# mathematiguy/pypardis

Measured on AMD Instinct MI355X. Metric: points clustered/sec (whole node), 100M 3-D pts, 1/2/4/8 GPUs; % HBM roofline, higher is better.
Workload: dtype f32 coords, f64 predicate

## Files before the change

### pypardis_amd/csrc/engine.hip

```cpp
#include <cstring>
#include <rocprim/rocprim.hpp>
#ifndef PD_SORT_ROCPRIM
#define PD_SORT_ROCPRIM 0
#endif

#include <algorithm>
#include <type_traits>
#include <cmath>
#include <cstring>
#include <vector>

#include "compact.hpp"
#include "internal.hpp"
#include "pred.hpp"
#include "rsort.hpp"
#include "scan.hpp"
#include "stream.hpp"
#include "uf.hpp"

namespace pd {
namespace {

#ifndef PD_CHECK_BOUNDS
#define PD_CHECK_BOUNDS 0
// ... 526 lines not shown
__global__ __launch_bounds__(kBlock) void cell_tile_kernel(const K* __restrict__ keys, uint64_t R,
                                                           uint32_t* __restrict__ tile_cnt) {
    uint32_t st[4];
    uint64_t kv[4];
    const uint64_t r0 = ((uint64_t)blockIdx.x * kBlock + threadIdx.x) * 4;
    const uint32_t t = block_sum_u32(cell_starts4<K>(keys, R, r0, st, kv));
    if (threadIdx.x == 0) tile_count_out(tile_cnt, t);
}

template <typename K>
__global__ __launch_bounds__(kBlock) void cell_write_kernel(const K* __restrict__ keys, uint64_t R,
                                                            const uint64_t* __restrict__ tile_off,
                                                            uint32_t* __restrict__ cstart,
                                                            K* __restrict__ ckeys,
                                                            uint32_t* __restrict__ ncells) {
    uint32_t st[4];
    uint64_t kv[4];
    const uint64_t r0 = ((uint64_t)blockIdx.x * kBlock + threadIdx.x) * 4;
    uint32_t btot;
    const uint32_t c = cell_starts4<K>(keys, R, r0, st, kv);
    uint32_t cid = (uint32_t)tile_off[blockIdx.x] + block_excl_scan(c, btot);
#pragma unroll
    for (int q = 0; q < 4; ++q) {
        if (st[q]) {
            cstart[cid] = (uint32_t)(r0 + q);
            ckeys[cid] = (K)kv[q];
        }
        cid += st[q];
        if (r0 + q == R - 1) {
            cstart[cid] = (uint32_t)R;
            *ncells = cid;
        }
    }
}

template <typename WT>
__device__ __forceinline__ WT shfl_up_w(WT x, int o) {
    if constexpr (sizeof(WT) == 4) return (WT)__shfl_up((int)x, o, 64);
    else return (WT)__shfl_up((long long)x, o, 64);
}
template <typename WT>
__device__ __forceinline__ WT shfl_down_w(WT x, int o) {
    if constexpr (sizeof(WT) == 4) return (WT)__shfl_down((int)x, o, 64);
    else return (WT)__shfl_down((long long)x, o, 64);
}
template <typename WT>
__device__ __forceinline__ WT shfl_w(WT x, int l) {
    if constexpr (sizeof(WT) == 4) return (WT)__shfl((int)x, l, 64);
    else return (WT)__shfl((long long)x, l, 64);
}

template <typename K, int SH, bool W32>
__global__ __launch_bounds__(kBlock) void dir_bits_kernel(const K* __restrict__ ckeys,
                                                          const uint32_t* __restrict__ ncells,
                                                          uint4* __restrict__ dir) {
    const uint32_t c = blockIdx.x * kBlock + threadIdx.x;
    const uint32_t nc = *ncells;
    if (c - (uint32_t)(threadIdx.x & 63) >= nc) return;
    const bool in = c < nc;
    using WT = std::conditional_t<W32, uint32_t, uint64_t>;
    const uint64_t k = in ? ((uint64_t)ckeys[c] >> SH) : ~0ull;
    const WT word = (WT)(k >> 6);
    unsigned long long v = in ? (1ull << (k & 63)) : 0ull;
    const int lane = threadIdx.x & 63;
#pragma unroll
    for (int o = 1; o < 64; o <<= 1) {
        const WT wo = shfl_up_w(word, o);
        const unsigned long long vo = (unsigned long long)__shfl_up((long long)v, o, 64);
        if (lane >= o && wo == word) v |= vo;
    }
    const WT wn = shfl_down_w(word, 1);
    const bool last = lane == 63 || wn != word;
    if (in && last) atomicOr(reinterpret_cast<unsigned long long*>(dir + (uint64_t)word), v);
}

template <typename K, bool W32>
__global__ __launch_bounds__(kBlock) void word_write_kernel(const K* __restrict__ ckeys,
                                                            const uint32_t* __restrict__ ncells,
                                                            const uint4* __restrict__ pages,
                                                            uint4* __restrict__ words) {
    const uint32_t c = blockIdx.x * kBlock + threadIdx.x;
    const uint32_t nc = *ncells;
    if (c - (uint32_t)(threadIdx.x & 63) >= nc) return;
    const bool in = c < nc;
    using WT = std::conditional_t<W32, uint32_t, uint64_t>;
    const uint64_t k = in ? (uint64_t)ckeys[c] : ~0ull;
    const WT word = (WT)(k >> 6);
    unsigned long long v = in ? (1ull << (k & 63)) : 0ull;
    const int lane = threadIdx.x & 63;
#pragma unroll
    for (int o = 1; o < 64; o <<= 1) {
        const WT wo = shfl_down_w(word, o);
        const unsigned long long vo = (unsigned long long)__shfl_down((long long)v, o, 64);
        if (lane + o < 64 && wo == word) v |= vo;
    }
    const WT wp = shfl_up_w(word, 1);
    const WT w63 = shfl_w(word, 63);
    const uint32_t cb = c - (uint32_t)lane;
    unsigned long long vx = 0;
    if (cb + 64 < nc && (WT)((uint64_t)ckeys[cb + 64] >> 6) == w63) {
        const uint32_t c2 = cb + 64 + (uint32_t)lane;
        const uint64_t k2 = c2 < nc ? (uint64_t)ckeys[c2] : ~0ull;
        vx = c2 < nc && (WT)(k2 >> 6) == w63 ? 1ull << (k2 & 63) : 0ull;
#pragma unroll
        for (int o = 32; o > 0; o >>= 1) vx |= (unsigned long long)__shfl_xor((long long)vx, o, 64);
    }
    if (!in) return;
    bool first = c == 0;
    if (!first) first = lane ? wp != word : (WT)((uint64_t)ckeys[c - 1] >> 6) != word;
    bool occ;
    const uint64_t slot = page_slot(pages[(uint64_t)word >> 6], (uint64_t)word, occ);
    if (first) {
        if (w63 == word) v |= vx;
        words[slot] = make_uint4((uint32_t)v, (uint32_t)(v >> 32), c, 0u);
    }
    if (c == nc - 1) words[slot + 1] = make_uint4(0u, 0u, nc, 0u);
}

__device__ __forceinline__ uint32_t dir_popc4(const uint4* __restrict__ dir, uint64_t W,
                                              uint64_t w0, uint32_t (&pc)[4]) {
    uint32_t t = 0;
#pragma unroll
    for (int q = 0; q < 4; ++q) {
        pc[q] = 0;
        if (w0 + q < W) {
            const uint4 d = dir[w0 + q];
            pc[q] = (uint32_t)__popc(d.x) + (uint32_t)__popc(d.y);
        }
        t += pc[q];
    }
    return t;
}

__global__ __launch_bounds__(kBlock) void dir_tile_kernel(const uint4* __restrict__ dir, uint64_t W,
                                                          uint32_t* __restrict__ tile_cnt) {
    uint32_t pc[4];
    const uint32_t t =
        block_sum_u32(dir_popc4(dir, W, ((uint64_t)blockIdx.x * kBlock + threadIdx.x) * 4, pc));
    if (threadIdx.x == 0) tile_count_out(tile_cnt, t);
}

__global__ __launch_bounds__(kBlock) void dir_write_kernel(uint4* __restrict__ dir, uint64_t W,
                                                           const uint64_t* __restrict__ tile_off) {
    uint32_t pc[4], btot;
    const uint64_t w0 = ((uint64_t)blockIdx.x * kBlock + threadIdx.x) * 4;
    uint32_t z = (uint32_t)tile_off[blockIdx.x] + block_excl_scan(dir_popc4(dir, W, w0, pc), btot);
#pragma unroll
    for (int q = 0; q < 4; ++q) {
        if (w0 + q < W) dir[w0 + q].z = z;
        z += pc[q];
    }
}

constexpr int kSubTiles = 4;
#ifndef PD_ROOTS_SUB
#define PD_ROOTS_SUB 4
#endif
constexpr int kRootSub = PD_ROOTS_SUB;
constexpr int kRootLists = 64, kRootCntStride = 32;
__global__ __launch_bounds__(kBlock) void init_kernel(uint32_t R, const uint8_t* __restrict__ core,
                                                      const uint32_t* __restrict__ mn,
                                                      int use_mn, uint32_t* __restrict__ par,
                                                      uint32_t* __restrict__ gmin,
                                                      uint32_t* __restrict__ wroot, uint64_t W,
                                                      uint32_t* __restrict__ kbits, uint64_t NW) {
#pragma unroll
    for (int q = 0; q < kSubTiles; ++q) {
        const uint64_t r64 = ((uint64_t)blockIdx.x * kSubTiles + q) * kBlock + threadIdx.x;
        if (r64 < W) wroot[r64] = kNone;
        if (r64 < NW) kbits[r64] = 0u;
        if (r64 >= R) continue;
        const uint32_t r = (uint32_t)r64;
        gmin[r] = kNone;
        uint32_t p = kNone;
        if (core[r] & 1) {
            p = r;
            if (use_mn) {
                const uint2 m = reinterpret_cast<const uint2*>(mn)[r];
                if (m.x < r && (core[m.x] & 1))
                    p = m.x;
                else if (m.y < r && (core[m.y] & 1))
                    p = m.y;
            }
        }
        par[r] = p;
    }
}

struct LinkStats {
    uint32_t cand = 0, hit = 0, core = 0, same = 0, find_same = 0, unions = 0;
};

__global__ __launch_bounds__(kBlock) void rep_kernel(const uint32_t* __restrict__ list,
                                                     const uint32_t* __restrict__ count,
                                                     const uint32_t* __restrict__ vals,
                                                     const uint32_t* __restrict__ par,
                                                     uint32_t* __restrict__ rep) {
    const uint32_t nl = *count;
    for (uint32_t i = blockIdx.x * kBlock + threadIdx.x; i < nl; i += gridDim.x * kBlock) {
        const uint32_t r = list[i];
        if (par[r] != kNone) atomicMin(rep + (vals[r] & kIdMask), r);
    }
}

__global__ __launch_bounds__(kBlock) void merge_kernel(const uint32_t* __restrict__ list,
                                                       const uint32_t* __restrict__ count,
                                                       const uint32_t* __restrict__ vals,
                                                       const uint32_t* __restrict__ rep,
                                                       uint32_t* __restrict__ par) {
    const uint32_t nl = *count;
    const int lane = threadIdx.x & 63;
    for (uint32_t b0 = blockIdx.x * kBlock; b0 < nl; b0 += gridDim.x * kBlock) {
        const uint32_t i = b0 + threadIdx.x;
        uint32_t ra = kNone, rb = kNone;
        if (i < nl) {
            const uint32_t r = list[i];
            if (ld_rlx(par + r) != kNone) {
                const uint32_t q = rep[vals[r] & kIdMask];
                if (q != r) {
                    ra = uf_find(par, r);
                    rb = uf_find(par, q);
                    if (ra > rb) {
                        const uint32_t t = ra;
                        ra = rb;
                        rb = t;
                    }
                    if (ra == rb) ra = rb = kNone;
                }
            }
        }
        const uint32_t pa = (uint32_t)__shfl_up((int)ra, 1, 64);
        const uint32_t pb = (uint32_t)__shfl_up((int)rb, 1, 64);
        const bool same = lane > 0 && pa == ra && pb == rb;
        if (ra != kNone && !same) uf_unite(par, ra, rb);
    }
}

__global__ __launch_bounds__(kBlock) void roots_kernel(uint32_t R, const uint32_t* __restrict__ vals,
                                                       const uint32_t* __restrict__ gid,
                                                       uint32_t* __restrict__ par,
                                                       uint32_t* __restrict__ gmin,
                                                       uint32_t* __restrict__ rlist,
                                                       uint32_t* __restrict__ rcnt, uint32_t seg,
                                                       uint32_t* __restrict__ counts, int stats) {
    uint32_t ncore = 0;
    uint32_t rr[kRootSub], x0[kRootSub], root[kRootSub], pt[kRootSub];
    bool core[kRootSub];
#pragma unroll
    for (int q = 0; q < kRootSub; ++q) {
        rr[q] = (blockIdx.x * kRootSub + q) * kBlock + threadIdx.x;
        x0[q] = rr[q] < R ? par[rr[q]] : kNone;
        core[q] = x0[q] != kNone;
    }
#pragma unroll
    for (int q = 0; q < kRootSub; ++q) {
        root[q] = core[q] ? par[x0[q]] : 0u;
        pt[q] = core[q] ? (vals[rr[q]] & kIdMask) : kNone;
    }
    bool more[kRootSub];
#pragma unroll
    for (int q = 0; q < kRootSub; ++q) more[q] = core[q] && root[q] != x0[q];
    while (true) {
        bool any = false;
#pragma unroll
        for (int q = 0; q < kRootSub; ++q) any |= more[q];
        if (!__any(any)) break;
        uint32_t p[kRootSub];
#pragma unroll
        for (int q = 0; q < kRootSub; ++q) p[q] = more[q] ? par[root[q]] : root[q];
#pragma unroll
        for (int q = 0; q < kRootSub; ++q) {
            if (p[q] == root[q]) more[q] = false;
            root[q] = p[q];
        }
    }
#pragma unroll
    for (int q = 0; q < kRootSub; ++q) {
        if (!core[q]) continue;
        if (root[q] != x0[q]) par[rr[q]] = root[q];
        if (gid) pt[q] = gid[pt[q]];
        ncore += 1u;
    }
    bool left[kRootSub];
#pragma unroll
    for (int q = 0; q < kRootSub; ++q) left[q] = core[q];
    while (true) {
        bool have = false;
        uint32_t key = 0, m = kNone;
#pragma unroll
        for (int q = 0; q < kRootSub; ++q) {
            if (left[q] && !have) {
                have = true;
                key = root[q];
            }
        }
#pragma unroll
        for (int q = 0; q < kRootSub; ++q) {
            if (left[q] && root[q] == key) {
                m = pt[q] < m ? pt[q] : m;
                left[q] = false;
            }
        }
        if (!__any(have)) break;
        wave_atomic_min(gmin, have, key, m);
    }
    if (rlist) {
        __shared__ uint32_t s_rbase;
        uint32_t nr = 0;
#pragma unroll
        for (int q = 0; q < kRootSub; ++q) nr += core[q] && root[q] == rr[q] ? 1u : 0u;
        uint32_t tot;
        uint32_t off = block_excl_scan(nr, tot);
        const uint32_t k = blockIdx.x % kRootLists;
        if (threadIdx.x == 0 && tot) s_rbase = atomicAdd(rcnt + k * kRootCntStride, tot);
        __syncthreads();
        if (tot) {
            uint32_t* out = rlist + (size_t)k * seg + s_rbase;
#pragma unroll
            for (int q = 0; q < kRootSub; ++q)
                if (core[q] && root[q] == rr[q]) out[off++] = rr[q];
        }
    }
    if (stats) {
        const uint32_t c = block_sum_u32(ncore);
        if (threadIdx.x == 0 && c) atomicAdd(counts + 1, c);
    }
}

__global__ __launch_bounds__(kBlock) void root_mark_kernel(const uint32_t* __restrict__ rlist,
                                                           const uint32_t* __restrict__ rcnt,
                                                           uint32_t seg,
                                                           const uint32_t* __restrict__ gmin,
                                                           uint32_t* __restrict__ kbits) {
    const uint32_t k = blockIdx.x % kRootLists, m = gridDim.x / kRootLists;
    const uint32_t c = rcnt[k * kRootCntStride];
    const uint32_t* l = rlist + (size_t)k * seg;
    for (uint32_t i = (blockIdx.x / kRootLists) * kBlock + threadIdx.x; i < c; i += m * kBlock) {
        const uint32_t g = gmin[l[i]];
// ... 1105 lines not shown
    const uint64_t t0 = (uint64_t)t * TILE;
    if (t0 >= c) return;
    const int tid = threadIdx.x;
    const int sb = kLabBits - kLabBitsL;
    const uint32_t nsub = 1u << sb, smask = nsub - 1;
    if (tid < kLabMaxSub) cnt[tid] = 0;
    __syncthreads();
    const uint2* src = pairs + ((uint64_t)b << kLabBits);
    uint2 q[PER];
    uint32_t lr[PER];
#pragma unroll
    for (int i = 0; i < PER; ++i) {
        const uint64_t k = t0 + (uint64_t)i * kLabBlock + tid;
        q[i] = make_uint2(kNone, kNone);
        if (k < c) {
            const unsigned long long w =
                __builtin_nontemporal_load(reinterpret_cast<const unsigned long long*>(src + k));
            q[i] = make_uint2((uint32_t)w, (uint32_t)(w >> 32));
        }
    }
#pragma unroll
    for (int i = 0; i < PER; ++i)
        lr[i] = q[i].x != kNone ? atomicAdd(&cnt[(q[i].x >> kLabBitsL) & smask], 1u) : 0u;
    __syncthreads();
    if (tid < 64) {
        const uint32_t v = (uint32_t)tid < nsub ? cnt[tid] : 0u;
        uint32_t x = v;
#pragma unroll
        for (int o = 1; o < 64; o <<= 1) {
            const uint32_t y = (uint32_t)__shfl_up((int)x, o, 64);
            if (tid >= o) x += y;
        }
        off[tid] = x - v;
        gbase[tid] = v ? atomicAdd(bcnt2 + ((uint64_t)b << sb) + tid, v) : 0u;
        if (tid == 63) s_total = x;
    }
    __syncthreads();
#pragma unroll
    for (int i = 0; i < PER; ++i)
        if (q[i].x != kNone) stage[off[(q[i].x >> kLabBitsL) & smask] + lr[i]] = q[i];
    __syncthreads();
    const uint32_t total = s_total;
    for (uint32_t p = tid; p < total; p += kLabBlock) {
        const uint2 v = stage[p];
        const uint32_t g = v.x >> kLabBitsL, u = g & smask;
        pairs2[((uint64_t)g << kLabBitsL) + gbase[u] + (p - off[u])] = v;
    }
}

__global__ __launch_bounds__(kLabBlock) void label_local_kernel(const uint2* __restrict__ pairs,
                                                                const uint32_t* __restrict__ bcnt,
                                                                uint64_t n,
                                                                int32_t* __restrict__ labels,
                                                                uint8_t* __restrict__ core_out) {
    constexpr uint32_t NB = 1u << kLabBitsL, MASK = NB - 1;
    __shared__ uint32_t img[NB];
    const uint32_t b = blockIdx.x;
    const int tid = threadIdx.x;
    for (uint32_t i = tid; i < NB; i += kLabBlock) img[i] = kNone;
    __syncthreads();
    const uint32_t c = bcnt[b];
    const unsigned long long* p =
        reinterpret_cast<const unsigned long long*>(pairs + ((uint64_t)b << kLabBitsL));
    constexpr int U = 4;
    for (uint32_t k0 = 0; k0 < c; k0 += U * kLabBlock) {
        unsigned long long w[U];
#pragma unroll
        for (int u = 0; u < U; ++u) {
            const uint32_t k = k0 + u * kLabBlock + tid;
            w[u] = k < c ? __builtin_nontemporal_load(p + k) : ~0ull;
        }
#pragma unroll
        for (int u = 0; u < U; ++u)
            if (k0 + u * kLabBlock + tid < c) img[(uint32_t)w[u] & MASK] = (uint32_t)(w[u] >> 32);
    }
    __syncthreads();
    const uint64_t base = (uint64_t)b << kLabBitsL;
    const uint32_t m = (uint32_t)std::min<uint64_t>(NB, n - base);
    for (uint32_t i = tid; i < m; i += kLabBlock) {
        const uint32_t k = img[i];
        labels[base + i] = k == kNone ? -1 : (int32_t)(k & ~kKeyCoreBit);
        if (core_out) core_out[base + i] = (k != kNone && (k & kKeyCoreBit)) ? 1 : 0;
    }
}

__global__ __launch_bounds__(kBlock) void final_label_kernel(const uint32_t* __restrict__ key,
                                                             uint64_t n, int32_t* __restrict__ labels,
                                                             uint8_t* __restrict__ core_out) {
    const uint64_t i = (uint64_t)blockIdx.x * kBlock + threadIdx.x;
    if (i >= n) return;
    const uint32_t k = key[i];
    labels[i] = k == kNone ? -1 : (int32_t)(k & ~kKeyCoreBit);
    if (core_out) core_out[i] = (k != kNone && (k & kKeyCoreBit)) ? 1 : 0;
}

__global__ __launch_bounds__(kBlock) void split_core_kernel(uint32_t* __restrict__ key, uint64_t n,
                                                            uint32_t mask,
                                                            uint8_t* __restrict__ core) {
    const uint64_t i = (uint64_t)blockIdx.x * kBlock + threadIdx.x;
    if (i >= n) return;
    const uint32_t k = key[i];
    const bool c = k != kNone && (k & mask);
    if (core) core[i] = c ? 1 : 0;
    if (c) key[i] = k & ~mask;
}

__device__ __forceinline__ uint32_t key_id(uint32_t k, int core_bit) {
    return (core_bit && k != kNone) ? (k & ~kKeyCoreBit) : k;
}

__global__ __launch_bounds__(kBlock) void root_flag_kernel(const uint32_t* __restrict__ key,
                                                           uint64_t n, int core_bit,
                                                           uint32_t* __restrict__ flag) {
    const uint64_t i = (uint64_t)blockIdx.x * kBlock + threadIdx.x;
    if (i < n) flag[i] = key_id(key[i], core_bit) == (uint32_t)i ? 1u : 0u;
}

__global__ __launch_bounds__(kBlock) void label_kernel(const uint32_t* __restrict__ key,
                                                       const uint32_t* __restrict__ rnk,
                                                       const uint32_t* __restrict__ flag,
                                                       uint64_t n, int core_bit,
                                                       int32_t* __restrict__ labels,
                                                       uint8_t* __restrict__ core_out,
                                                       int64_t* __restrict__ ncl) {
    const uint64_t i = (uint64_t)blockIdx.x * kBlock + threadIdx.x;
    if (i >= n) return;
    const uint32_t k = key[i];
    const uint32_t id = key_id(k, core_bit);
    labels[i] = k == kNone ? -1 : (int32_t)rnk[id];
    if (core_bit && core_out) core_out[i] = (k != kNone && (k & kKeyCoreBit)) ? 1 : 0;
    if (i == n - 1) *ncl = (int64_t)rnk[i] + flag[i];
}

struct EvTimer {
    Ctx& ctx;
    hipStream_t s;
    int k = 0;
    explicit EvTimer(Ctx& c, hipStream_t st) : ctx(c), s(st) {}
    void mark() {
        if (!ctx.timing) return;
        if (!ctx.ev[k]) PD_HIP(hipEventCreate(&ctx.ev[k]));
        PD_HIP(hipEventRecord(ctx.ev[k], s));
        ++k;
    }
    float span(int a, int b) {
        if (!ctx.timing || b >= k) return 0;
        float ms = 0;
        PD_HIP(hipEventElapsedTime(&ms, ctx.ev[a], ctx.ev[b]));
        return ms;
    }
};

inline unsigned blocks(uint64_t n) { return n ? (unsigned)((n + kBlock - 1) / kBlock) : 1u; }
inline unsigned sub_blocks(uint64_t n, int sub = kSubTiles) {
    return n ? (unsigned)((n + (uint64_t)kBlock * sub - 1) / ((uint64_t)kBlock * sub)) : 1u;
}

uint64_t tile_offsets(Ctx& ctx, uint32_t* cnt, unsigned tiles, uint64_t* off, hipStream_t s,
                      bool read_total) {
    size_t tb = 0;
    PD_HIP(rocprim::exclusive_scan(nullptr, tb, cnt, off, (uint64_t)0, (size_t)tiles + 1,
                                   rocprim::plus<uint64_t>(), s));
    void* tmp = ctx.arena.get<char>("tile_scan_tmp", tb);
    PD_HIP(rocprim::exclusive_scan(tmp, tb, cnt, off, (uint64_t)0, (size_t)tiles + 1,
                                   rocprim::plus<uint64_t>(), s));
    if (!read_total) return 0;
    uint64_t* h = (uint64_t*)pinned(ctx, sizeof(uint64_t));
    PD_HIP(hipMemcpyAsync(h, off + tiles, sizeof(uint64_t), hipMemcpyDeviceToHost, s));
    sync(s);
    return *h;
}
inline int xsub_of(const Ctx& ctx) { return ctx.xsub < 1 ? 1 : ctx.xsub; }

template <typename T, int D, int M, bool ST>
void launch_count(hipStream_t s, const T* Xs, uint32_t R, const Cells& C, double eps, double eps2,
                  float lo, float hi, uint32_t ms, int full, uint32_t rot_min, uint8_t* core,
                  uint32_t* mn, uint32_t* cnt, unsigned long long* st) {
    if constexpr (ST)
        hipLaunchKernelGGL((count4_kernel<T, D, M, true, 1>), dim3(blocks(R)), dim3(kBlock), 0, s,
                           Xs, R, C, eps, eps2, lo, hi, ms, full, rot_min, core, mn, cnt, st, 0u);
    else
        hipLaunchKernelGGL((count4_kernel<T, D, M, false, kCountWpe>), dim3(blocks(R)), dim3(kBlock), 0, s,
                           Xs, R, C, eps, eps2, lo, hi, ms, full, rot_min, core, mn, cnt, st, 0u);
}

#ifndef PD_WCOUNT_WPE
#define PD_WCOUNT_WPE 0
#endif
template <int D>
constexpr int kWCountWpe = PD_WCOUNT_WPE ? PD_WCOUNT_WPE : (D <= 2 ? 8 : (D == 3 ? 6 : 5));
template <typename T, int D, int M>
void launch_count_weighted(hipStream_t s, const T* Xs, uint32_t R, const Cells& C, double eps,
                           double eps2, float lo, float hi, uint32_t ms, int full,
                           uint32_t rot_min, uint8_t* core, uint32_t* mn, const uint64_t* wrec) {
    hipLaunchKernelGGL((count4_kernel<T, D, M, false, kWCountWpe<D>, false, true>), dim3(blocks(R)),
                       dim3(kBlock), 0, s, Xs, R, C, eps, eps2, lo, hi, ms, full, rot_min, core, mn,
                       (uint32_t*)nullptr, (unsigned long long*)nullptr, 0u, wrec,
                       (uint64_t)ms << kWeightFrac);
}

template <typename T, int D, int M>
float replay_count(hipStream_t s, const T* Xs, uint32_t R, uint32_t reps, const Cells& C,
                   double eps, double eps2, float lo, float hi, uint32_t ms, int full,
                   uint32_t rot_min, uint8_t* core, uint32_t* mn, uint32_t* cnt) {
    const uint64_t RL = (uint64_t)R * reps;
    if (RL >= 0xFFFFFFFFull) throw Error(-1, "count replay: more than 2^32 - 1 lanes");
    hipEvent_t e0, e1;
    PD_HIP(hipEventCreate(&e0));
    PD_HIP(hipEventCreate(&e1));
    PD_HIP(hipEventRecord(e0, s));
    hipLaunchKernelGGL((count4_kernel<T, D, M, false, kCountWpe, true>), dim3(blocks(RL)), dim3(kBlock), 0,
                       s, Xs, (uint32_t)RL, C, eps, eps2, lo, hi, ms, full, rot_min, core, mn, cnt,
                       (unsigned long long*)nullptr, R);
    PD_HIP(hipEventRecord(e1, s));
    PD_HIP(hipEventSynchronize(e1));
    float msec = 0;
    PD_HIP(hipEventElapsedTime(&msec, e0, e1));
    (void)hipEventDestroy(e0);
    (void)hipEventDestroy(e1);
    return msec;
}

template <typename T, int D, int M>
void launch_border(hipStream_t s, const T* Xs, uint32_t NL, const uint32_t* list, const Cells& C,
                   double eps, double eps2, float lo, float hi, const uint32_t* vals,
                   const uint32_t* par, const uint32_t* gmin, uint32_t* key_out,
                   uint32_t* rec_out = nullptr) {
    hipLaunchKernelGGL((border4_kernel<T, D, M, kBorderWpe>), dim3(blocks(NL)), dim3(kBlock), 0, s, Xs, NL,
                       list, C, eps, eps2, lo, hi, vals, par, gmin, key_out, rec_out);
}

template <typename K>
void sort_records(Ctx& ctx, K*& keys, uint32_t*& vals, K* keys2, uint32_t* vals2, uint64_t R,
                  int key_bits, hipStream_t s, bool hist_zeroed) {
#if PD_SORT_ROCPRIM
    rocprim::double_buffer<K> kb(keys, keys2);
    rocprim::double_buffer<uint32_t> vb(vals, vals2);
    size_t tb = 0;
    PD_HIP(rocprim::radix_sort_pairs(nullptr, tb, kb, vb, (size_t)R, 0u, (unsigned)key_bits, s));
    void* tmp = ctx.arena.get<char>("sort_tmp", tb);
    PD_HIP(rocprim::radix_sort_pairs(tmp, tb, kb, vb, (size_t)R, 0u, (unsigned)key_bits, s));
    keys = kb.current();
    vals = vb.current();
#else
    const uint64_t tiles = rsort::tiles_for(R, (int)sizeof(K));
    const uint64_t want = std::max<uint64_t>(tiles, ctx.rs_look_tiles);
    uint64_t* look = ctx.arena.get<uint64_t>("rsort_look", want * rsort::kRadix);
    if (look != ctx.rs_look || want > ctx.rs_look_tiles) {
        PD_HIP(hipMemsetAsync(look, 0, sizeof(uint64_t) * rsort::kRadix * want, s));
        ctx.rs_look = look;
        ctx.rs_look_tiles = want;
        ctx.rs_epoch = 0;
    }
    rsort::State st;
    st.look = look;
    st.look_tiles = ctx.rs_look_tiles;
    st.hist = ctx.arena.get<uint32_t>("rsort_hist", 8 * rsort::kRadix);
    st.ticket = ctx.arena.get<unsigned long long>("rsort_ticket", 1);
    st.epoch = ctx.rs_epoch;
    K* ko;
    uint32_t* vo;
    rsort::sort_pairs<K>(st, keys, vals, keys2, vals2, R, key_bits, s, &ko, &vo, hist_zeroed);
    ctx.rs_epoch = st.epoch;
    keys = ko;
    vals = vo;
#endif
}

template <typename Pred>
uint32_t select_records(Ctx& ctx, const char* name, uint32_t R, Pred pred, uint32_t** out,
                        hipStream_t s) {
    uint32_t* list = ctx.arena.get<uint32_t>(name, R);
    *out = list;
    return (uint32_t)compact_ordered(ctx, "sel_cmp", (uint64_t)R, pred, list, nullptr, s);
}

void check_bounds(hipStream_t s, const char* kernel) {
#if PD_CHECK_BOUNDS
    unsigned long long h[2] = {0, 0};
    PD_HIP(hipStreamSynchronize(s));
    PD_HIP(hipMemcpyFromSymbol(h, HIP_SYMBOL(g_oob), sizeof(h), 0, hipMemcpyDeviceToHost));
    if (h[0]) {
        const unsigned long long z[2] = {0, 0};
        PD_HIP(hipMemcpyToSymbol(HIP_SYMBOL(g_oob), z, sizeof(z), 0, hipMemcpyHostToDevice));
        throw Error(-1, std::string("bounds check failed in ") + kernel + ": " +
                            std::to_string(h[0]) + " violation(s), first at site " +
                            std::to_string(h[1] >> 48) + " index " +
                            std::to_string(h[1] & 0xFFFFFFFFFFFFull));
    }
#else
    (void)s;
    (void)kernel;
#endif
}

template <typename T, int D, typename K, int M>
void run_a(Ctx& ctx, TrainArgs& a, const std::vector<PartGrid>& hparts, uint64_t Gtot,
           int key_bits, EvTimer& tm) {
    hipStream_t s = a.stream;
    const uint64_t n = (uint64_t)a.n;
    const int P = a.P;
    if (Gtot >= (1ull << 53)) throw Error(-5, "eps grid of 2^53 cells or more");
    tm.mark();

    PartGrid* parts = ctx.arena.get<PartGrid>("parts", P);
    const T* X = (const T*)a.X;

// ... 71 lines not shown
                       (uint64_t)R, parts, P, part_start);
    uint32_t* cstart = ctx.arena.get<uint32_t>("cstart", (size_t)R + 1);
    K* ckeys = ctx.arena.get<K>("cell_keys", (size_t)R + 1);
    uint32_t* dncells = ctx.arena.get<uint32_t>("ncells", 4);
    if (R) {
        const unsigned ctiles = (unsigned)((R + 4 * kBlock - 1) / (4 * kBlock));
        uint32_t* ccnt = ctx.arena.get<uint32_t>("tile_cnt", (size_t)ctiles + 1);
        uint64_t* coff = ctx.arena.get<uint64_t>("tile_off", (size_t)ctiles + 1);
        hipLaunchKernelGGL((cell_tile_kernel<K>), dim3(ctiles), dim3(kBlock), 0, s, keys,
                           (uint64_t)R, ccnt);
        tile_offsets(ctx, ccnt, ctiles, coff, s, false);
        hipLaunchKernelGGL((cell_write_kernel<K>), dim3(ctiles), dim3(kBlock), 0, s, keys,
                           (uint64_t)R, coff, cstart, ckeys, dncells);
    } else {
        PD_HIP(hipMemsetAsync(cstart, 0, sizeof(uint32_t), s));
        PD_HIP(hipMemsetAsync(dncells, 0, sizeof(uint32_t), s));
    }
    uint64_t cgrid0 = R;
#if PD_NC_SYNC
    if (R) {
        uint32_t* hnc = (uint32_t*)((char*)pinned(ctx, 16) + 8);
        PD_HIP(hipMemcpyAsync(hnc, dncells, sizeof(uint32_t), hipMemcpyDeviceToHost, s));
        uint32_t* hwb = hnc + 1;
        if (wbad) PD_HIP(hipMemcpyAsync(hwb, wbad, sizeof(uint32_t), hipMemcpyDeviceToHost, s));
        sync(s);
        cgrid0 = std::max<uint64_t>(1, std::min<uint64_t>(*hnc, R));
        if (wbad && *hwb)
            throw Error(-1, "sample_weight: " + std::to_string(*hwb) +
                                " value(s) not finite or outside [0, 2^31]");
        wbad = nullptr;
    }
#endif
    if (wbad) {
        uint32_t* hwb = (uint32_t*)pinned(ctx, sizeof(uint32_t));
        PD_HIP(hipMemcpyAsync(hwb, wbad, sizeof(uint32_t), hipMemcpyDeviceToHost, s));
        sync(s);
        if (*hwb)
            throw Error(-1, "sample_weight: " + std::to_string(*hwb) +
                                " value(s) not finite or outside [0, 2^31]");
    }
    auto prefix_words = [&](uint4* d, uint64_t nw, bool read_total) -> uint64_t {
        const unsigned wtiles = (unsigned)std::max<uint64_t>(1, (nw + 4 * kBlock - 1) / (4 * kBlock));
        uint32_t* wcnt = ctx.arena.get<uint32_t>("tile_cnt", (size_t)wtiles + 1);
        uint64_t* woff = ctx.arena.get<uint64_t>("tile_off", (size_t)wtiles + 1);
        hipLaunchKernelGGL(dir_tile_kernel, dim3(wtiles), dim3(kBlock), 0, s, d, nw, wcnt);
        const uint64_t tot = tile_offsets(ctx, wcnt, wtiles, woff, s, read_total);
        hipLaunchKernelGGL(dir_write_kernel, dim3(wtiles), dim3(kBlock), 0, s, d, nw, woff);
        return tot;
    };
    uint64_t W;
    uint4* dir;
    uint4* pages = nullptr;
    if (!a.dir_paged) {
        W = (Gtot >> 6) + 2;
        dir = ctx.arena.get<uint4>("dir", W);
        PD_HIP(hipMemsetAsync(dir, 0, sizeof(uint4) * W, s));
        if (R) {
            if (sizeof(K) == 4 || key_bits <= 37)
                hipLaunchKernelGGL((dir_bits_kernel<K, 0, true>), dim3(blocks(cgrid0)), dim3(kBlock), 0, s,
                                   ckeys, dncells, dir);
            else
                hipLaunchKernelGGL((dir_bits_kernel<K, 0, false>), dim3(blocks(cgrid0)), dim3(kBlock), 0,
                                   s, ckeys, dncells, dir);
        }
        prefix_words(dir, W, false);
    } else {
        const uint64_t NP = (Gtot >> 12) + 2;
        pages = ctx.arena.get<uint4>("dir_pages", NP);
        PD_HIP(hipMemsetAsync(pages, 0, sizeof(uint4) * NP, s));
        if (R) {
            if (sizeof(K) == 4 || key_bits <= 43)
                hipLaunchKernelGGL((dir_bits_kernel<K, 6, true>), dim3(blocks(cgrid0)), dim3(kBlock), 0, s,
                                   ckeys, dncells, pages);
            else
                hipLaunchKernelGGL((dir_bits_kernel<K, 6, false>), dim3(blocks(cgrid0)), dim3(kBlock), 0,
                                   s, ckeys, dncells, pages);
        }
        if (R && !PD_NC_SYNC)
            PD_HIP(hipMemcpyAsync((char*)pinned(ctx, 16) + 8, dncells, sizeof(uint32_t),
                                  hipMemcpyDeviceToHost, s));
        const uint64_t nw = prefix_words(pages, NP, true);
        W = nw + 1;
        dir = ctx.arena.get<uint4>("dir", W);
        if (R)
        {
            const uint32_t nch = *(const uint32_t*)((const char*)pinned(ctx, 16) + 8);
            const uint64_t wg = std::max<uint64_t>(1, std::min<uint64_t>(nch, R));
            if (sizeof(K) == 4 || key_bits <= 37)
                hipLaunchKernelGGL((word_write_kernel<K, true>), dim3(blocks(wg)), dim3(kBlock), 0, s,
                                   ckeys, dncells, pages, dir);
            else
                hipLaunchKernelGGL((word_write_kernel<K, false>), dim3(blocks(wg)), dim3(kBlock), 0, s,
                                   ckeys, dncells, pages, dir);
        }
        else
            PD_HIP(hipMemsetAsync(dir, 0, sizeof(uint4), s));
    }
    ctx.t.dir_words = (int64_t)W;
    PD_HIP(hipGetLastError());
    tm.mark();

    Cells C{parts, part_start, P, dir, cstart, pages};
    const double eps = a.eps, eps2 = a.eps * a.eps;
    float slo = -1.0f, shi = INFINITY;
    {
        const double thr = a.metric == 0 ? eps2 : eps;
        if (std::is_same<T, float>::value && thr > 1e-30 && thr < 1e30 && ctx.screen) {
            slo = std::nextafter((float)(thr * (1.0 - 1.0 / 262144.0)), 0.0f);
            shi = std::nextafter((float)(thr * (1.0 + 1.0 / 262144.0)), INFINITY);
        }
    }
    uint8_t* core = ctx.arena.get<uint8_t>("core", R);
    uint32_t* mn = ctx.arena.get<uint32_t>("minnbr", 2 * (size_t)R);
    uint32_t* cnt_rec = a.counts ? ctx.arena.get<uint32_t>("cnt_rec", R) : nullptr;
    unsigned long long* sst = nullptr;
    if (ctx.sweep_stats) {
        sst = ctx.arena.get<unsigned long long>("sweep_stats", 10);
        PD_HIP(hipMemsetAsync(sst, 0, sizeof(unsigned long long) * 10, s));
    }
    uint32_t* h_nc = nullptr;
    hipEvent_t ev_nc = nullptr;
    if (R && ctx.centre_window < 0) {
        h_nc = (uint32_t*)pinned(ctx, sizeof(uint32_t));
        PD_HIP(hipEventCreateWithFlags(&ev_nc, hipEventDisableTiming));
        PD_HIP(hipMemcpyAsync(h_nc, dncells, sizeof(uint32_t), hipMemcpyDeviceToHost, s));
        PD_HIP(hipEventRecord(ev_nc, s));
    }
    if (R) {
        const uint32_t rot = ctx.count_rotate ? (uint32_t)ctx.count_rotate : 0xFFFFFFFFu;
        if (wrec)
            launch_count_weighted<T, D, M>(s, Xs, R, C, eps, eps2, slo, shi, (uint32_t)a.min_samples,
                                           ctx.full_counts ? 1 : 0, rot, core, mn, wrec);
        else if (sst)
            launch_count<T, D, M, true>(s, Xs, R, C, eps, eps2, slo, shi, (uint32_t)a.min_samples,
                                        ctx.full_counts ? 1 : 0, rot, core, mn, cnt_rec, sst);
        else
            launch_count<T, D, M, false>(s, Xs, R, C, eps, eps2, slo, shi, (uint32_t)a.min_samples,
                                         ctx.full_counts ? 1 : 0, rot, core, mn, cnt_rec, sst);
        if (ctx.count_replay > 0 && !sst && !wrec)
            ctx.t.count_kernel = replay_count<T, D, M>(
                s, Xs, R, (uint32_t)ctx.count_replay, C, eps, eps2, slo, shi,
                (uint32_t)a.min_samples, ctx.full_counts ? 1 : 0, rot, core, mn, cnt_rec);
    }
    PD_HIP(hipGetLastError());
    tm.mark();

    uint32_t* par = ctx.arena.get<uint32_t>("parent", R);
    uint32_t* gmin = ctx.arena.get<uint32_t>("gmin", R);
    if (R) {
        uint32_t* wroot = ctx.arena.get<uint32_t>("word_root", W);
        const uint64_t NW = a.phase == 0 ? (n + 31) / 32 : 0;
        const uint64_t NWz = NW ? ((NW + 31) & ~uint64_t(31)) + kRootLists * kRootCntStride : 0;
        uint32_t* kbits = NW ? ctx.arena.get<uint32_t>("key_bits", NWz) : nullptr;
        hipLaunchKernelGGL(init_kernel, dim3(sub_blocks(std::max<uint64_t>(std::max<uint64_t>(R, W), NWz))),
                           dim3(kBlock), 0, s, R, core, mn, 1, par, gmin, wroot, (uint64_t)W, kbits, NWz);
        int cw = ctx.centre_window;
        uint64_t cgrid = R;
        if (cw < 0) {
            PD_HIP(hipEventSynchronize(ev_nc));
            (void)hipEventDestroy(ev_nc);
            const uint32_t nc = *h_nc ? *h_nc : 1u;
            cgrid = std::min<uint64_t>(nc, R);
            cw = 2 * (uint64_t)R <= 5ull * nc ? 2 : ((uint64_t)R <= 8ull * nc ? 8 : 16);
        }
        auto go = [&](auto Wc) {
            constexpr int Wv = decltype(Wc)::value;
            constexpr int Kw = window_groups((int)sizeof(T), D, Wv);
            const unsigned wb = blocks(((uint64_t)R + Kw - 1) / Kw);
            if (sst)
                hipLaunchKernelGGL((window_uf_kernel<T, D, M, Wv, true>), dim3(wb), dim3(kBlock), 0,
                                   s, Xs, R, eps, eps2, slo, shi, par, sst);
            else
                hipLaunchKernelGGL((window_uf_kernel<T, D, M, Wv, false>), dim3(wb), dim3(kBlock), 0,
                                   s, Xs, R, eps, eps2, slo, shi, par, sst);
        };
        if (cw <= 2)
            go(std::integral_constant<int, 2>{});
        else if (cw <= 4)
            go(std::integral_constant<int, 4>{});
        else if (cw <= 8)
            go(std::integral_constant<int, 8>{});
        else if (cw <= 16)
            go(std::integral_constant<int, 16>{});
        else if (cw <= 32)
            go(std::integral_constant<int, 32>{});
        else
            go(std::integral_constant<int, 64>{});
        uint32_t* croot = ctx.arena.get<uint32_t>("cell_root", R);
        {
            uint32_t* big = ctx.arena.get<uint32_t>("big_cells", R / (kWordBig + 1) + 1);
            uint32_t* mid = ctx.arena.get<uint32_t>("mid_cells", R / (kMidCell + 1) + 1);
            uint32_t* nbig = ctrs + 8;
            if ((uint64_t)W < 0xFFFFFFFFull)
                hipLaunchKernelGGL((cell_word_root_kernel<K, true>), dim3(blocks(cgrid)), dim3(kBlock), 0,
                                   s, cstart, dncells, ckeys, par, croot, wroot, mid, nbig + 1, big,
                                   nbig, pages);
            else
                hipLaunchKernelGGL((cell_word_root_kernel<K, false>), dim3(blocks(cgrid)), dim3(kBlock),
                                   0, s, cstart, dncells, ckeys, par, croot, wroot, mid, nbig + 1,
                                   big, nbig, pages);
            hipLaunchKernelGGL((mid_cell_word_root_kernel<K>), dim3(2048), dim3(kBlock), 0, s,
                               cstart, ckeys, mid, nbig + 1, par, croot, wroot, pages);
            hipLaunchKernelGGL((big_cell_word_root_kernel<K>), dim3(1024), dim3(kBlock), 0, s,
                               cstart, ckeys, big, nbig, par, croot, wroot, pages);
        }
        const uint32_t pcap = (uint32_t)std::min<uint64_t>(R, 64ull << 20);
        uint2* plist = ctx.arena.get<uint2>("pair_list", pcap);
        uint32_t* pcount = ctrs + 10;
        const unsigned vtiles = blocks(cgrid);
        uint8_t* vflag = ctx.arena.get<uint8_t>("verify_flags", R);
        uint32_t* vlist = ctx.arena.get<uint32_t>("verify_list", R);
        uint32_t* vcnt = ctx.arena.get<uint32_t>("tile_cnt", (size_t)vtiles + 1);
        uint64_t* voff = ctx.arena.get<uint64_t>("tile_off", (size_t)vtiles + 1);
        if (ctx.verify_fused) {
            hipLaunchKernelGGL((cell_verify_kernel<T, D, M, K>), dim3(vtiles), dim3(kBlock), 0, s,
                               Xs, keys, nullptr, 0u, croot, wroot, C, xsub_of(ctx), eps, eps2,
                               slo, shi, par, plist, pcap, pcount, sst, dncells);
        } else {
            hipLaunchKernelGGL((verify_screen_kernel<D, K>), dim3(vtiles), dim3(kBlock), 0, s, keys,
                               dncells, croot, wroot, C, xsub_of(ctx), vflag, vcnt);
            const uint32_t NV = (uint32_t)tile_offsets(ctx, vcnt, vtiles, voff, s, true);
            if (NV) {
                hipLaunchKernelGGL(flag_list_kernel, dim3(vtiles), dim3(kBlock), 0, s, vflag, dncells,
                                   voff, vlist);
                hipLaunchKernelGGL((cell_verify_kernel<T, D, M, K>), dim3(blocks(NV)), dim3(kBlock), 0,
                                   s, Xs, keys, vlist, NV, croot, wroot, C, xsub_of(ctx), eps, eps2,
                                   slo, shi, par, plist, pcap, pcount, sst, nullptr);
            }
        }
        hipLaunchKernelGGL((pair_kernel<T, D, M>), dim3(std::min(blocks(pcap), 4096u)), dim3(kBlock), 0, s, Xs, plist,
                           pcount, pcap, cstart, croot, eps, eps2, slo, shi, par);
    }
    PD_HIP(hipGetLastError());
    tm.mark();
    if (P > 1 && R) {
        const unsigned gb = std::min(blocks(R), 2048u);
        hipLaunchKernelGGL(rep_kernel, dim3(gb), dim3(kBlock), 0, s, dup_list, lcount, vals, par,
                           rep);
        hipLaunchKernelGGL(merge_kernel, dim3(gb), dim3(kBlock), 0, s, dup_list, lcount, vals, rep,
                           par);
    }
    tm.mark();
    if (R) {
        const unsigned rb = sub_blocks(R, kRootSub);
        const uint32_t seg = ((rb + kRootLists - 1) / kRootLists) * (uint32_t)(kRootSub * kBlock);
        const uint64_t NW = a.phase == 0 ? (n + 31) / 32 : 0;
        uint32_t* rlist = NW ? ctx.arena.get<uint32_t>("root_list", (size_t)seg * kRootLists) : nullptr;
        uint32_t* rcnt = NW ? ctx.arena.get<uint32_t>("key_bits", 1) + ((NW + 31) & ~uint64_t(31))
                            : nullptr;
        hipLaunchKernelGGL(roots_kernel, dim3(rb), dim3(kBlock), 0, s, R, vals, a.gid, par, gmin, rlist,
                           rcnt, seg, lcount + 1, ctx.sweep_stats ? 1 : 0);
        if (a.phase == 0) {
            uint32_t* kbits = ctx.arena.get<uint32_t>("key_bits", 1);
            uint32_t* kpre = ctx.arena.get<uint32_t>("key_pre", NW);
            const unsigned gb = kRootLists * 16;
            hipLaunchKernelGGL(root_mark_kernel, dim3(gb), dim3(kBlock), 0, s, rlist, rcnt, seg, gmin,
                               kbits);
            rocprim::transform_iterator<const uint32_t*, PopcOp, uint32_t> pc(kbits, PopcOp{});
            size_t tb = 0;
            PD_HIP(rocprim::exclusive_scan(nullptr, tb, pc, kpre, 0u, (size_t)NW,
                                           rocprim::plus<uint32_t>(), s));
            void* tmp = ctx.arena.get<char>("key_scan_tmp", tb);
            PD_HIP(rocprim::exclusive_scan(tmp, tb, pc, kpre, 0u, (size_t)NW,
                                           rocprim::plus<uint32_t>(), s));
            hipLaunchKernelGGL(root_rank_kernel, dim3(gb), dim3(kBlock), 0, s, rlist, rcnt, seg, kbits,
                               kpre, NW, gmin, lcount + 1);
        } else if (ctx.sweep_stats) {
            uint32_t* h = (uint32_t*)pinned(ctx, sizeof(uint32_t) * 4);
            PD_HIP(hipMemcpyAsync(h, lcount + 2, sizeof(uint32_t), hipMemcpyDeviceToHost, s));
            sync(s);
            ctx.t.core_records = h[0];
        }
    }
    ctx.st.n_roots = 0;
    PD_HIP(hipGetLastError());
    tm.mark();

    PhaseState& st = ctx.st;
    st.R = R;
    st.n = n;
    st.G = Gtot;
    st.P = P;
    st.d = D;
    st.dtype = std::is_same<T, float>::value ? 0 : 1;
    st.metric = M;
    st.min_samples = a.min_samples;
    st.key_bits = key_bits;
    st.eps = a.eps;
    st.slo = slo;
    st.shi = shi;
    st.Xs = Xs;
    st.parts = parts;
    st.part_start = part_start;
    st.dir = dir;
    st.pages = pages;
    st.cstart = cstart;
    st.vals = vals;
    st.core = core;
    st.par = par;
    st.gmin = gmin;
    st.cnt_rec = cnt_rec;
    st.mn = mn;
    st.n_exports = 0;
    if (a.phase == 1 && R && a.xr) {
        uint32_t* elist = nullptr;
        const uint32_t NE = select_records(ctx, "export_list", R, IsExport{core, vals, a.xr},
                                           &elist, s);
        st.exp_gid = ctx.arena.get<uint32_t>("exp_gid", NE + 1);
// ... 452 lines not shown
```

Measured before the change: 4.309 billion.

## Compress parent pointers within each init tile using shared-memory pointer jumping

The init kernel now handles 16 sub-tiles per block and stages each row's initial parent in LDS. Within a tile it iterates pointer jumping until every parent either points outside the tile or reaches a fixed point, then writes the compressed parents to global memory. This is meant to shorten the union-find trees before the later link and find phases, so they do fewer global-memory hops. The cost is a larger static LDS footprint, lower occupancy and extra barrier-synchronised loops in init. The launch grid shrinks to match the larger tile.

```diff
diff --git a/pypardis_amd/csrc/engine.hip b/pypardis_amd/csrc/engine.hip
--- a/pypardis_amd/csrc/engine.hip
+++ b/pypardis_amd/csrc/engine.hip
@@ -702,7 +702,12 @@
     }
 }
 
-constexpr int kSubTiles = 4;
+#ifndef PD_INIT_SUB
+#define PD_INIT_SUB 16
+#endif
+constexpr int kInitSub = PD_INIT_SUB;
+constexpr uint32_t kInitTile = (uint32_t)kInitSub * kBlock;
+static_assert(kInitSub >= 1 && kInitTile * 4 <= 65536, "a block's static LDS");
 #ifndef PD_ROOTS_SUB
 #define PD_ROOTS_SUB 4
 #endif
@@ -714,26 +719,70 @@
                                                       uint32_t* __restrict__ gmin,
                                                       uint32_t* __restrict__ wroot, uint64_t W,
                                                       uint32_t* __restrict__ kbits, uint64_t NW) {
-#pragma unroll
-    for (int q = 0; q < kSubTiles; ++q) {
-        const uint64_t r64 = ((uint64_t)blockIdx.x * kSubTiles + q) * kBlock + threadIdx.x;
+    __shared__ uint32_t lp[kInitTile];
+    const uint64_t base = (uint64_t)blockIdx.x * kInitTile;
+    uint32_t p[kInitSub];
+#pragma unroll
+    for (int q = 0; q < kInitSub; ++q) {
+        const uint32_t e = (uint32_t)q * kBlock + threadIdx.x;
+        const uint64_t r64 = base + e;
         if (r64 < W) wroot[r64] = kNone;
         if (r64 < NW) kbits[r64] = 0u;
-        if (r64 >= R) continue;
-        const uint32_t r = (uint32_t)r64;
-        gmin[r] = kNone;
-        uint32_t p = kNone;
-        if (core[r] & 1) {
-            p = r;
-            if (use_mn) {
-                const uint2 m = reinterpret_cast<const uint2*>(mn)[r];
-                if (m.x < r && (core[m.x] & 1))
-                    p = m.x;
-                else if (m.y < r && (core[m.y] & 1))
-                    p = m.y;
+        p[q] = kNone;
+        if (r64 < R) {
+            const uint32_t r = (uint32_t)r64;
+            gmin[r] = kNone;
+            if (core[r] & 1) {
+                p[q] = r;
+                if (use_mn) {
+                    const uint2 m = reinterpret_cast<const uint2*>(mn)[r];
+                    if (m.x < r && (core[m.x] & 1))
+                        p[q] = m.x;
+                    else if (m.y < r && (core[m.y] & 1))
+                        p[q] = m.y;
+                }
             }
         }
-        par[r] = p;
+        lp[e] = p[q];
+    }
+    if (base >= R) return;
+    const uint32_t b32 = (uint32_t)base;
+    uint32_t open = 0;
+#pragma unroll
+    for (int q = 0; q < kInitSub; ++q) {
+        const uint32_t e = (uint32_t)q * kBlock + threadIdx.x;
+        if (p[q] != kNone && p[q] != b32 + e && p[q] >= b32) open |= 1u << q;
+    }
+    __syncthreads();
+    while (true) {
+        uint32_t g[kInitSub];
+#pragma unroll
+        for (int q = 0; q < kInitSub; ++q) {
+            g[q] = p[q];
+            if ((open >> q & 1u) && PD_OK(p[q] - b32 < kInitTile, 9, p[q]))
+                g[q] = __hip_atomic_load(lp + (p[q] - b32), __ATOMIC_RELAXED,
+                                         __HIP_MEMORY_SCOPE_WORKGROUP);
+        }
+        int moved = 0;
+#pragma unroll
+        for (int q = 0; q < kInitSub; ++q) {
+            if (!(open >> q & 1u)) continue;
+            if (g[q] == p[q] || g[q] == kNone) {
+                open &= ~(1u << q);
+                continue;
+            }
+            p[q] = g[q];
+            __hip_atomic_store(lp + ((uint32_t)q * kBlock + threadIdx.x), g[q], __ATOMIC_RELAXED,
+                               __HIP_MEMORY_SCOPE_WORKGROUP);
+            moved = 1;
+            if (g[q] < b32) open &= ~(1u << q);
+        }
+        if (!__syncthreads_or(moved)) break;
+    }
+#pragma unroll
+    for (int q = 0; q < kInitSub; ++q) {
+        const uint64_t r64 = base + (uint32_t)q * kBlock + threadIdx.x;
+        if (r64 < R) par[r64] = p[q];
     }
 }
 
@@ -2145,7 +2194,7 @@
 };
 
 inline unsigned blocks(uint64_t n) { return n ? (unsigned)((n + kBlock - 1) / kBlock) : 1u; }
-inline unsigned sub_blocks(uint64_t n, int sub = kSubTiles) {
+inline unsigned sub_blocks(uint64_t n, int sub) {
     return n ? (unsigned)((n + (uint64_t)kBlock * sub - 1) / ((uint64_t)kBlock * sub)) : 1u;
 }
 
@@ -2523,8 +2572,10 @@
         const uint64_t NW = a.phase == 0 ? (n + 31) / 32 : 0;
         const uint64_t NWz = NW ? ((NW + 31) & ~uint64_t(31)) + kRootLists * kRootCntStride : 0;
         uint32_t* kbits = NW ? ctx.arena.get<uint32_t>("key_bits", NWz) : nullptr;
-        hipLaunchKernelGGL(init_kernel, dim3(sub_blocks(std::max<uint64_t>(std::max<uint64_t>(R, W), NWz))),
+        hipLaunchKernelGGL(init_kernel,
+                           dim3(sub_blocks(std::max<uint64_t>(std::max<uint64_t>(R, W), NWz), kInitSub)),
                            dim3(kBlock), 0, s, R, core, mn, 1, par, gmin, wroot, (uint64_t)W, kbits, NWz);
+        check_bounds(s, "init_kernel");
         int cw = ctx.centre_window;
         uint64_t cgrid = R;
         if (cw < 0) {
```

Result: faster. 4.433 billion (median of 6 runs) (+2.9%).
